# rvp-group/srrg2_proslam

Measured on AMD Instinct MI355X. Metric: tracked frames/sec on KITTI-00 stereo (1241x376, ~2k kp); SE(3) vs ref, higher is better.
Workload: dtype u64 popcount (Hamming) + f32 (projection, Jacobians, 6x6 normal equations)

## Files before the change

srrg2_proslam_amd/csrc/align.hip:

```cpp
#include "prs_device.h"
#include "prs_host.h"
#include "prs_se3.h"

#include <math.h>
#include <string.h>

#include <type_traits>
#include <vector>

namespace prs {

constexpr int kAlignThreads = 256;
constexpr int kTerms        = 29;
constexpr uint32_t kNoneU32 = 0xffffffffu;
constexpr float kFltMax     = 3.402823466e+38f;

typedef unsigned int au32x4 __attribute__((ext_vector_type(4)));

struct AlignShared {
  float X[16];
  float A[16];
  float Sinv[16];
  float T[16];
  float Tprev[16];
// ... 17 lines not shown

static_assert(offsetof(AlignShared, b) == offsetof(AlignShared, H) + 36 * sizeof(float) && offsetof(AlignShared, chi_in) == offsetof(AlignShared, b) + 6 * sizeof(float) &&
                offsetof(AlignShared, chi_tot) == offsetof(AlignShared, chi_in) + sizeof(float),
              "the summed slots are written through AlignShared::H");

struct FrameCtl {
  int it_align;
  int need_search;
  int done;
  int executed;
  int flags;
  int n_inl, n_out, n_inv;
  int db_ready;
};
constexpr int kModeSplitSearch = 100;
constexpr int kSearchThreads   = 512;

struct AlignArgs {
  prs_pcf_params f;
  prs_aligner_params a;
  prs_align_batch b;
  int mode;
  int no_prefilter;
  int surv_slots;
  int narrow_prefilter_limit;
  int rows_table;
  int lut_cap;
  int cell_sy, cell_sx, cell_ncx, cell_ncy, ncells;
  float4* ops;
  FrameCtl* ctl;
  int* pending;
  unsigned char* dbcache;
  uint32_t db_blob;
  unsigned long long* stamps;
  int max_fixed;
  uint32_t off_db, off_inv, off_cellstart, off_cfix, off_cmov, off_cls, off_sh;
  const float* prior_mean;
  uint32_t off_u;
  uint32_t off_fdesc, off_fuv, off_best, off_second, off_lut, off_surv;
  uint32_t off_terms;
};

enum { kDecisionCommit = 0, kDecisionRetry = 1, kDecisionReturn = 2 };



__device__ __forceinline__ int isqrt_exact(int n) {
  int s = (int) sqrtf((float) n);
  while (s * s > n) {
    --s;
  }
  while ((s + 1) * (s + 1) <= n) {
    ++s;
  }
  return s;
}

__device__ __forceinline__ int hamming_regs(const au32x4& a0, const au32x4& a1, const au32x4& b0, const au32x4& b1) {
  uint32_t d = (uint32_t) __popc(a0.x ^ b0.x);
  d = popc_acc(a0.y ^ b0.y, d);
  d = popc_acc(a0.z ^ b0.z, d);
  d = popc_acc(a0.w ^ b0.w, d);
  d = popc_acc(a1.x ^ b1.x, d);
  d = popc_acc(a1.y ^ b1.y, d);
  d = popc_acc(a1.z ^ b1.z, d);
  d = popc_acc(a1.w ^ b1.w, d);
  return (int) d;
}

__device__ __forceinline__ int cold_copy(int v) {
  asm volatile("" : "+v"(v));
  return v;
}

__device__ __forceinline__ int hamming_half(const au32x4& a0, const au32x4& b0) {
  uint32_t d = (uint32_t) __popc(a0.x ^ b0.x);
  d = popc_acc(a0.y ^ b0.y, d);
  d = popc_acc(a0.z ^ b0.z, d);
  d = popc_acc(a0.w ^ b0.w, d);
  return (int) d;
}
__device__ __forceinline__ int hamming_96(const au32x4& a0, const au32x4& b0) {
  uint32_t d = (uint32_t) __popc(a0.x ^ b0.x);
  d = popc_acc(a0.y ^ b0.y, d);
  d = popc_acc(a0.z ^ b0.z, d);
  return (int) d;
}

__device__ __forceinline__ int irrelevant_distance(const float dd, const float ratio) {
  if (!(dd > 0.0f) || !(ratio > 0.0f) || !(dd <= 256.0f)) {
    return 0;
  }
  const int r_max = (int) ceilf(dd) - 1;
  if (r_max <= 0) {
    return 1;
  }
  float guess = (float) r_max / ratio;
  int b       = guess < 1024.0f ? (int) guess : 1024;
  b           = b > r_max ? b : r_max + 1;
  while (b < 2048 && !((float) r_max / (float) b < ratio)) {
    ++b;
  }
  return b < 2048 ? b : 0;
}

// ... 330 lines not shown
    sh.chi_in = sh.chi_tot = 0.0f;
    sh.mean_disp           = (split_search && ctl->it_align != 0) ? gres->mean_disparity : g.a.mean_disparity;
    sh.corr_changed        = 1;
    sh.have_terms          = 0;
    sh.have_cls            = 0;
    if (sh.n_corr < 0 || sh.n_corr > nF) {
      sh.n_corr = 0;
    }
    {
      float x[16], a16[16], si[16];
      const float* gx = g.b.X + (size_t) frame * 16;
#pragma unroll
      for (int i = 0; i < 16; ++i) {
        x[i] = gx[i];
      }
      se3_inverse(g.a.sensor_in_robot, si);
      pose_to_camera(g.a, si, x, a16);
#pragma unroll
      for (int i = 0; i < 16; ++i) {
        sh.Sinv[i] = si[i];
        sh.A[i]    = a16[i];
      }
    }
    if (nF > g.max_fixed) {
      sh.error = PRS_ERR_CAPACITY;
    }
  }
  for (int i = tid; i < 36; i += T) {
    sh.H[i] = 0.0f;
  }
  if (tid < 6) {
    sh.b[tid] = 0.0f;
  }
  __syncthreads();

  bool inputs_changed = g.b.inputs_changed ? (g.b.inputs_changed[frame] != 0) : true;
  if (split_search && ctl->it_align != 0) {
    inputs_changed = false;
  }
  bool db_built       = false;
  if (inputs_changed && g.mode != PRS_MODE_LINEARIZE) {
    if (tid == 0) {
      sh.n_corr = 0;
    }
    __syncthreads();
  }

  if (g.mode != PRS_MODE_FINDER && (!split_search || ctl->it_align == 0) && g.a.factor_type == PRS_FACTOR_STEREO &&
      g.a.enable_inverse_depth_weighting && g.a.mean_disparity < 0.0f && !sh.error) {
    for (int i = tid; i < nF; i += T) {
      const float4 c = gfix[i];
      terms[i]       = c.x - c.z;
    }
    __syncthreads();
    if (tid == 0) {
      float acc = 0.0f;
      int i     = 0;
      const float4* t4 = reinterpret_cast<const float4*>(terms);
      float4 n0 = t4[0], n1 = t4[1], n2 = t4[2], n3 = t4[3];
      for (; i + 16 <= nF; i += 16) {
        const float4 q0 = n0, q1 = n1, q2 = n2, q3 = n3;
        const int k = (i >> 2) + 4;
        n0 = t4[k];
        n1 = t4[k + 1];
        n2 = t4[k + 2];
        n3 = t4[k + 3];
        acc += q0.x; acc += q0.y; acc += q0.z; acc += q0.w;
        acc += q1.x; acc += q1.y; acc += q1.z; acc += q1.w;
        acc += q2.x; acc += q2.y; acc += q2.z; acc += q2.w;
        acc += q3.x; acc += q3.y; acc += q3.z; acc += q3.w;
      }
      for (; i < nF; ++i) {
        acc += terms[i];
      }
      sh.mean_disp = nF > 0 ? acc / (float) (size_t) nF : 0.0f;
    }
    __syncthreads();
  }

  if (g.mode != PRS_MODE_FINDER && !split_search && !sh.error) {
    for (int c = tid; c < sh.n_corr; c += T) {
      const prs_corr cr = gcorr[c];
      if (cr.fixed_idx < 0 || cr.fixed_idx >= nF || cr.moving_idx < 0 || cr.moving_idx >= nM) {
        sh.error = PRS_ERR_RANGE;
      } else {
        cfix[c] = gfix[cr.fixed_idx];
        cmov[c] = gmov[cr.moving_idx];
      }
    }
    __syncthreads();
  }

  enum { acc_finder = 0, acc_lin, acc_sum, acc_solve, acc_db, acc_search, acc_pass2, acc_filter, acc_commit };
  if (g.stamps && tid == 0) {
    for (int i = 0; i < 9; ++i) {
      sh.stamp_acc[i] = 0;
    }
    sh.stamp_mark = sh.stamp_sub = 0;
  }
#define SUB_MARK() do { if (g.stamps && tid == 0) { sh.stamp_sub = (unsigned long long) clock64(); } } while (0)
#define SUB_ACC(v) do { if (g.stamps && tid == 0) { const unsigned long long now_ = (unsigned long long) clock64(); sh.stamp_acc[v] += now_ - sh.stamp_sub; sh.stamp_sub = now_; } } while (0)
#define ALIGN_MARK() do { if (g.stamps && tid == 0) { sh.stamp_mark = (unsigned long long) clock64(); } } while (0)
#define ALIGN_ACC(v) do { if (g.stamps && tid == 0) { sh.stamp_acc[v] += (unsigned long long) clock64() - sh.stamp_mark; } } while (0)
  const int max_it = (g.mode == PRS_MODE_ALIGN && !sh.error) ? g.a.max_iterations + inlier_run_length(g.a) : (sh.error ? 0 : 1);
  if (split_search && sh.error && tid == 0) {
    ctl->done = 1;
  }
  int executed     = 0;
  int it_align     = 0;
  bool ran_inlier_phase = false;
// ... 9 lines not shown
    ALIGN_MARK();
    if (g.mode != PRS_MODE_LINEARIZE && !inlier_run) {
      if (tid < 16) {
        sh.T[tid] = sh.A[tid];
      }
      __syncthreads();
      for (;;) {
        const bool reset = inputs_changed || sh.config_changed;
        __syncthreads();
        if (reset) {
          if (tid == 0) {
            if ((sh.radius == 0 && sh.dd == 0.0f) || sh.config_changed) {
              sh.radius = g.f.maximum_search_radius_pixels;
              sh.dd     = g.f.minimum_descriptor_distance;
            }
            if (sh.config_changed) {
              sh.no_prune = 0;
            }
            sh.converged = 0;
            sh.it        = 0;
            se3_identity(sh.Tprev);
            sh.config_changed = 0;
            sh.kd_range       = (float) sh.radius;
          }
          inputs_changed = false;
          db_built       = false;
          __syncthreads();
        }
        if (sh.error) {
          break;
        }

        if (tid == 0) {
          sh.decision = kDecisionCommit;
          if (sh.converged) {
            sh.decision = kDecisionReturn;
          } else {
            float cam[16];
            se3_inverse(sh.T, cam);
            const unsigned long long k = g.f.number_of_solver_iterations_per_projection;
            if (k == 0 || sh.it % k == 0 || sh.it == 1) {
              se3_inverse(cam, sh.W);
              float delta[16], v6[6];
              se3_mul(cam, sh.Tprev, delta);
              t2tnq(delta, v6);
              sh.change_norm =
                sqrtf(((((v6[0] * v6[0] + v6[1] * v6[1]) + v6[2] * v6[2]) + v6[3] * v6[3]) + v6[4] * v6[4]) + v6[5] * v6[5]);
#pragma unroll
              for (int i = 0; i < 16; ++i) {
                sh.Tprev[i] = sh.T[i];
              }
              sh.n_projected = 0;
              sh.n_overflow  = 0;
              ++sh.num_recomputes;
            } else {
#pragma unroll
              for (int i = 0; i < 16; ++i) {
                sh.Tprev[i] = sh.T[i];
              }
              ++sh.it;
              sh.decision = kDecisionReturn;
            }
          }
        }
        __syncthreads();
        if (sh.decision == kDecisionReturn) {
          break;
        }

        SUB_MARK();
        if (!db_built && split_search && g.dbcache && ctl->db_ready) {
          const uint4* src = reinterpret_cast<const uint4*>(g.dbcache + (size_t) frame * g.db_blob);
          uint4* dst       = reinterpret_cast<uint4*>(smem + g.off_db);
          for (int i = tid; i < (int) (g.db_blob >> 4); i += T) {
            dst[i] = src[i];
          }
          __syncthreads();
          db_built = true;
        }
        if (!db_built && !lattice) {
          const int tid = cold_copy(tid_hot), lane = tid & 63, wave = tid >> 6;
          (void) lane;
          (void) wave;
          KdNode* nodes        = reinterpret_cast<KdNode*>(db);
          uint16_t* order      = inv;
          short* kdhead        = reinterpret_cast<short*>(cellstart);
          uint16_t* leaf_start = cellstart + 2;
          const int node_cap   = (int) ((size_t) g.max_fixed * sizeof(uint2) / sizeof(KdNode));
          const int open_cap   = kd_open_capacity(g.max_fixed);
          const int min_points = g.f.minimum_number_of_points_per_cluster > 0 ? g.f.minimum_number_of_points_per_cluster : 10;
          unsigned long long* st = reinterpret_cast<unsigned long long*>(terms);
          int* cnt        = reinterpret_cast<int*>(st + (size_t) open_cap * 5);
          int* kind       = cnt + open_cap;
          int* child_open = kind + open_cap;
          int* par_cur    = child_open + open_cap;
          int* pcnt_cur   = par_cur + open_cap;
          int* par_next   = pcnt_cur + open_cap;
          int* pcnt_next  = par_next + open_cap;
          uint16_t* node_of = reinterpret_cast<uint16_t*>(pcnt_next + open_cap);
          uint16_t* leaf_of = node_of + g.max_fixed + 2;
          uint16_t* bucket  = leaf_of + g.max_fixed + 2;
          for (int i = tid; i < nF; i += T) {
            const float4 c = gfix[i];
// ... 158 lines not shown
          __syncthreads();
          for (int i = tid; i < nF; i += T) {
            bucket[leaf_start[leaf_of[i]] + node_of[i]] = (uint16_t) i;
          }
          __syncthreads();
          for (int i = tid; i < nF; i += T) {
            const int l0 = leaf_start[leaf_of[i]], l1 = leaf_start[leaf_of[i] + 1];
            int rank = 0;
            for (int j = l0; j < l1; ++j) {
              rank += bucket[j] < (uint16_t) i ? 1 : 0;
            }
            order[l0 + rank] = (uint16_t) i;
          }
          if (tid == 0) {
            kdhead[1] = (short) n_leaves;
          }
          __syncthreads();
          db_built = true;
          if (split_search && g.dbcache) {
            const uint4* src = reinterpret_cast<const uint4*>(smem + g.off_db);
            uint4* dst       = reinterpret_cast<uint4*>(g.dbcache + (size_t) frame * g.db_blob);
            for (int i = tid; i < (int) (g.db_blob >> 4); i += T) {
              dst[i] = src[i];
            }
            if (tid == 0) {
              ctl->db_ready = 1;
            }
          }
        }
        if (!db_built) {
          const int tid = cold_copy(tid_hot), lane = tid & 63, wave = tid >> 6;
          (void) lane;
          (void) wave;
          const int histcap  = (R > g.ncells ? R : g.ncells) + 2;
          uint32_t* hist     = reinterpret_cast<uint32_t*>(terms);
          uint16_t* slot     = reinterpret_cast<uint16_t*>(hist + histcap);
          uint16_t* bucket   = slot + g.max_fixed + 2;
          uint16_t* canon    = bucket + g.max_fixed + 2;
          uint16_t* rowfirst = canon + g.max_fixed + 2;
          for (int i = tid; i <= R; i += T) {
            hist[i] = 0;
          }
          __syncthreads();
          for (int i = tid; i < nF; i += T) {
            const float4 c = gfix[i];
            if (c.x >= 0.0f && c.x < 32767.0f && c.y >= 0.0f && c.y < (float) R) {
              const int row = (int) (int16_t) c.y;
              slot[i]       = (uint16_t) atomicAdd(&hist[row], 1u);
            } else {
              sh.error = PRS_ERR_RANGE;
            }
          }
          __syncthreads();
          if (sh.error) {
            break;
          }
          {
            if (wave == 0) {
              const int n     = R + 1;
              const int chunk = (n + 63) >> 6;
              uint32_t sum    = 0;
              for (int j = 0; j < chunk; ++j) {
                const int r = lane * chunk + j;
                sum += r < n ? hist[r] : 0u;
              }
              uint32_t incl = sum;
#pragma unroll
              for (int d = 1; d < 64; d <<= 1) {
                const uint32_t o = __shfl_up(incl, d, 64);
                if (lane >= d) {
                  incl += o;
                }
              }
              uint32_t run = incl - sum;
              for (int j = 0; j < chunk; ++j) {
                const int r = lane * chunk + j;
                if (r < n) {
                  rowfirst[r] = (uint16_t) run;
                  run += hist[r];
                }
              }
            }
            __syncthreads();
            for (int i = tid; i < nF; i += T) {
              const int row = (int) (int16_t) gfix[i].y;
              bucket[rowfirst[row] + slot[i]] = (uint16_t) i;
            }
            __syncthreads();
            for (int i = tid; i < nF; i += T) {
              const int row = (int) (int16_t) gfix[i].y;
              const int s = rowfirst[row], e = rowfirst[row + 1];
              int rank = 0;
              for (int j = s; j < e; ++j) {
                rank += bucket[j] < (uint16_t) i ? 1 : 0;
              }
              canon[i] = (uint16_t) (s + rank);
            }
          }
          __syncthreads();
          for (int i = tid; i <= g.ncells; i += T) {
            hist[i] = 0;
          }
          __syncthreads();
          for (int i = tid; i < nF; i += T) {
            const float4 c = gfix[i];
            const int row  = (int) (int16_t) c.y;
            int cxi        = ((int) (int16_t) c.x) >> g.cell_sx;
            cxi            = cxi < g.cell_ncx ? cxi : g.cell_ncx - 1;
            slot[i]        = (uint16_t) atomicAdd(&hist[(row >> g.cell_sy) * g.cell_ncx + cxi], 1u);
          }
          __syncthreads();
          if (wave == 0) {
            const int n     = g.ncells + 1;
            const int chunk = (n + 63) >> 6;
            uint32_t sum    = 0;
            for (int j = 0; j < chunk; ++j) {
              const int r = lane * chunk + j;
              sum += r < n ? hist[r] : 0u;
            }
            uint32_t incl = sum;
#pragma unroll
            for (int d = 1; d < 64; d <<= 1) {
              const uint32_t o = __shfl_up(incl, d, 64);
              if (lane >= d) {
                incl += o;
              }
            }
            uint32_t run = incl - sum;
            for (int j = 0; j < chunk; ++j) {
              const int r = lane * chunk + j;
              if (r < n) {
                cellstart[r] = (uint16_t) run;
                run += hist[r];
              }
            }
          }
          __syncthreads();
          for (int i = tid; i < nF; i += T) {
            const float4 c = gfix[i];
            const int row  = (int) (int16_t) c.y;
            const int col  = (int) (int16_t) c.x;
            int cxi        = col >> g.cell_sx;
            cxi            = cxi < g.cell_ncx ? cxi : g.cell_ncx - 1;
            db[cellstart[(row >> g.cell_sy) * g.cell_ncx + cxi] + slot[i]] =
              make_uint2(((uint32_t) row & 0xffffu) | ((uint32_t) col << 16), (uint32_t) i | ((uint32_t) canon[i] << 16));
            inv[canon[i]] = (uint16_t) i;
          }
          if (tid == 0) {
            db[nF] = make_uint2(0x7fff7fffu, 0xffffffffu);
          }
          __syncthreads();
          db_built = true;
          if (split_search && g.dbcache) {
            const uint4* src = reinterpret_cast<const uint4*>(smem + g.off_db);
            uint4* dst       = reinterpret_cast<uint4*>(g.dbcache + (size_t) frame * g.db_blob);
            for (int i = tid; i < (int) (g.db_blob >> 4); i += T) {
              dst[i] = src[i];
            }
            if (tid == 0) {
              ctl->db_ready = 1;
            }
          }
        }

        SUB_ACC(acc_db);
        const int rad = (int) sh.radius;
        {
          const int tid = cold_copy(tid_hot);
          for (int i = tid; i < nF; i += T) {
            bestkey[i] = kNoneU32;
            second[i]  = kNoneU32;
          }
          if (lattice) {
            for (int pos = tid; pos < nF; pos += T) {
              const int fi  = (int) (db[pos].y & 0xffffu);
              fdesc[pos]    = gfd[2 * fi];
              fdesc_hi[pos] = gfd[2 * fi + 1];
            }
          } else {
            for (int i = tid; i < 2 * nF; i += T) {
              (i & 1 ? fdesc_hi : fdesc)[i >> 1] = gfd[i];
            }
            for (int i = tid; i < nF; i += T) {
              const float4 c = gfix[i];
              fuv[i]         = make_float2(c.x, c.y);
            }
          }
          if (stype == PRS_SEARCH_CIRCLE) {
            for (int i = tid; i < 2 * rad + 1 && i < g.lut_cap; i += T) {
              const int h = i - rad;
              lut[i]      = (uint16_t) (isqrt_exact(rad * rad - h * h) + 1);
            }
          }
        }
        __syncthreads();
        SUB_ACC(acc_pass2);
        {
          const float W0 = sh.W[0], W1 = sh.W[1], W2 = sh.W[2], W3 = sh.W[3];
          const float W4 = sh.W[4], W5 = sh.W[5], W6 = sh.W[6], W7 = sh.W[7];
          const float W8 = sh.W[8], W9 = sh.W[9], W10 = sh.W[10], W11 = sh.W[11];
          const float cols = (float) g.f.projector.canvas_cols, rows = (float) g.f.projector.canvas_rows;
          const float max_dd = g.f.maximum_descriptor_distance;
          const float r2f    = (float) (sh.radius * sh.radius);
          const int rad2     = rad * rad;
          const int irrelevant = irrelevant_distance(sh.dd, g.f.maximum_distance_ratio_to_second_best);
          const int prune_at   = (lattice && irrelevant > 0 && irrelevant <= 54 && !g.no_prefilter && !sh.no_prune) ? irrelevant : 0;
          const bool circle_exact = rad < 8192 && R + rad < 32000 && (g.cell_ncx << g.cell_sx) + rad < 32000;
          int projected      = 0;
          constexpr int kPre = SPLIT ? 1 : 4;
          for (int m0 = tid; m0 < nM; m0 += kPre * T) {
// ... 188 lines not shown
              if (bestk != kNoneU32) {
                cd.x = (lattice ? (uint32_t) inv[bestk & 0xffffu] : (bestk & 0xffffu)) | ((bestk >> 16) << 16);
                if (lattice && seck != kNoneU32) {
                  cd.y = (uint32_t) inv[seck & 0xffffu] | ((seck >> 16) << 16);
                }
              }
              auto emit = [&](const uint32_t c, const uint32_t tag) {
                const uint32_t f   = c & 0xffffu;
                const uint32_t key = ((c >> 16) << 17) | ((uint32_t) m << 1) | tag;
                const uint32_t old = atomicMin(&bestkey[f], key);
                if (old != kNoneU32) {
                  atomicMin(&second[f], (old > key ? old : key) >> 17);
                }
              };
              if (cd.x != kNoneU32) {
                emit(cd.x, 0u);
              }
              if (cd.y != kNoneU32) {
                emit(cd.y, 1u);
              }
            }
           }
          }
          if (projected) {
            atomicAdd(&sh.n_projected, projected);
          }
        }
        __syncthreads();
        SUB_ACC(acc_search);
        {
          const float ratio = g.f.maximum_distance_ratio_to_second_best;
          const float dd    = sh.dd;
          int base          = 0;
          for (int f0 = 0; f0 < nF; f0 += T) {
            const int f = f0 + tid;
            bool acc    = false;
            if (f < nF) {
              const uint32_t bk = bestkey[f];
              if (bk != kNoneU32) {
                const float resp = (float) (bk >> 17);
                const uint32_t s = second[f];
                const float fs   = s == kNoneU32 ? kFltMax : (float) s;
                acc = resp < dd && resp / fs < ratio && (bk & 1u) == 0u;
              }
            }
            const unsigned long long bal = __ballot(acc);
            const int pre                = __popcll(bal & ((1ull << lane) - 1ull));
            if (lane == 0) {
              sh.wave_tot[wave] = __popcll(bal);
            }
            __syncthreads();
            int wbase = base;
            for (int w = 0; w < wave; ++w) {
              wbase += sh.wave_tot[w];
            }
            if (f < nF) {
              second[f] = acc ? (uint32_t) (wbase + pre) : kNoneU32;
            }
            for (int w = 0; w < T / 64; ++w) {
              base += sh.wave_tot[w];
            }
            __syncthreads();
          }
          if (tid == 0) {
            sh.n_filtered = base;
          }
        }
        __syncthreads();
        if (tid == 0) {
          if (sh.n_projected == 0) {
            sh.flags |= PRS_WARN_NO_PROJECTION;
          }
          if (8 * sh.n_overflow > sh.n_projected) {
            sh.no_prune = 1;
          }
          const float matching_ratio = (float) sh.n_filtered / (float) (size_t) nF;
          sh.decision                = kDecisionCommit;
          if (matching_ratio < g.f.minimum_matching_ratio) {
            sh.flags |= PRS_WARN_LOW_RATIO;
            if (sh.radius < g.f.maximum_search_radius_pixels || sh.dd > g.f.minimum_descriptor_distance) {
              sh.radius = g.f.maximum_search_radius_pixels;
              sh.dd     = g.f.minimum_descriptor_distance;
              sh.flags |= PRS_WARN_RETRIED;
              if (matching_ratio == 0.0f) {
                sh.flags |= PRS_WARN_TRACK_LOST;
                se3_identity(sh.T);
                sh.it = 0;
              } else {
                ++sh.it;
              }
              sh.decision = kDecisionRetry;
            }
          }
          if (sh.decision == kDecisionCommit) {
            sh.n_corr       = sh.n_filtered;
            sh.corr_changed = 1;
            if (sh.change_norm < g.f.maximum_estimate_change_norm_for_convergence &&
                sh.it > g.f.minimum_number_of_iterations) {
              sh.converged = 1;
              if (matching_ratio > g.f.minimum_matching_ratio) {
                const unsigned long long reduced = sh.radius - g.f.search_radius_step_size_pixels;
                sh.radius = reduced > g.f.minimum_search_radius_pixels ? reduced : g.f.minimum_search_radius_pixels;
                const float increased = sh.dd + g.f.descriptor_distance_step_size_pixels;
                sh.dd = increased < g.f.maximum_descriptor_distance ? increased : g.f.maximum_descriptor_distance;
              }
            }
            ++sh.it;
          }
        }
        __syncthreads();
        if (sh.decision == kDecisionRetry) {
          continue;
        }
        SUB_ACC(acc_filter);
        for (int f = cold_copy(tid_hot); f < nF; f += T) {
          const uint32_t slot = second[f];
          if (slot != kNoneU32) {
            const uint32_t bk = bestkey[f];
            const int m       = (int) ((bk >> 1) & 0xffffu);
            prs_corr cr;
            cr.fixed_idx  = f;
            cr.moving_idx = m;
            cr.response   = (float) (bk >> 17);
            gcorr[slot]   = cr;
            if (g.mode == PRS_MODE_ALIGN) {
              cfix[slot] = gfix[f];
              cmov[slot] = gmov[m];
            }
          }
        }
        __syncthreads();
        SUB_ACC(acc_commit);
        break;
      }
      if (sh.error) {
        break;
      }
      if (tid == 0 && sh.n_corr == 0) {
        sh.flags |= PRS_WARN_NO_MATCHES;
      }
      __syncthreads();
    }
    ALIGN_ACC(acc_finder);
    if (g.mode == PRS_MODE_FINDER || split_search) {
      break;
    }

    const int nc = sh.n_corr;
    __syncthreads();
    if (g.mode == PRS_MODE_ALIGN && nc < g.a.min_num_correspondences) {
      if (tid == 0) {
        sh.n_inl = sh.n_out = sh.n_inv = 0;
        sh.chi_in = sh.chi_tot = 0.0f;
        sh.have_cls = 0;
      }
      for (int i = tid; i < 36; i += T) {
        sh.H[i] = 0.0f;
      }
      if (tid < 6) {
        sh.b[tid] = 0.0f;
      }
      __syncthreads();
      if (g.a.stop_at_fixed_point && (sh.converged || inlier_run)) {
        ran_inlier_phase = ran_inlier_phase || (inlier_run_length(g.a) > 0 && 0 >= g.a.min_num_inliers);
        break;
      }
      continue;
    }
    {
      const PoseRegs pose  = {sh.A[0], sh.A[1], sh.A[2], sh.A[3], sh.A[4], sh.A[5], sh.A[6], sh.A[7], sh.A[8], sh.A[9], sh.A[10], sh.A[11]};
      const float mean_dsp = sh.mean_disp;
      const bool pose_ok   = __all(pose_is_finite(pose));
      if (tid == 0) {
        sh.have_cls = 1;
// ... 86 lines not shown
      if (g.a.enable_motion_prior) {
        add_motion_prior(g.a, g.prior_mean ? g.prior_mean + (size_t) frame * 16 : nullptr, X, H, b);
      }
      float dx6[6];
      const bool step_ok = gn_step(H, b, g.a.damping, X, g.a.damping_form == PRS_DAMPING_IDENTITY, dx6);
      const float dn2 = ((((dx6[0] * dx6[0] + dx6[1] * dx6[1]) + dx6[2] * dx6[2]) + dx6[3] * dx6[3]) + dx6[4] * dx6[4]) + dx6[5] * dx6[5];
      const bool small_step = g.a.step_norm_exit > 0.0f && step_ok && dn2 < g.a.step_norm_exit * g.a.step_norm_exit;
      uint32_t changed_bits = 0;
#pragma unroll
      for (int i = 0; i < 16; ++i) {
        changed_bits |= __float_as_uint(X[i]) ^ __float_as_uint(sh.X[i]);
        sh.X[i] = X[i];
      }
      float a16[16];
      pose_to_camera(g.a, sh.Sinv, X, a16);
#pragma unroll
      for (int i = 0; i < 16; ++i) {
        sh.A[i] = a16[i];
      }
      sh.decision = ((g.a.stop_at_fixed_point && changed_bits == 0u && (sh.converged || inlier_run)) || (small_step && (sh.converged || inlier_run))) ? 1 : 0;
    }
    __syncthreads();
    ALIGN_ACC(acc_solve);
    if (sh.decision) {
      if (!inlier_run && inlier_run_length(g.a) > 0) {
        it_align = g.a.max_iterations - 1;
        continue;
      }
      ++it_align;
      break;
    }
  }

  __syncthreads();
  if (g.mode == PRS_MODE_ALIGN && !split_search && g.a.keep_only_inlier_correspondences && sh.have_cls && !sh.error) {
    const int nc = sh.n_corr;
    int base     = 0;
    for (int c0 = 0; c0 < nc; c0 += T) {
      const int c     = c0 + tid;
      const bool keep = c < nc && clsbuf[c] == 0;
      prs_corr cr;
      if (keep) {
        cr = gcorr[c];
      }
      const unsigned long long bal = __ballot(keep);
      if (lane == 0) {
        sh.wave_tot[wave] = __popcll(bal);
      }
      __syncthreads();
      int pos = base + __popcll(bal & ((1ull << lane) - 1ull));
      for (int w = 0; w < T / 64; ++w) {
        pos += w < wave ? sh.wave_tot[w] : 0;
        base += sh.wave_tot[w];
      }
      if (keep) {
        gcorr[pos] = cr;
      }
      __syncthreads();
    }
    if (tid == 0) {
      sh.n_corr = base;
    }
    __syncthreads();
  }

  __syncthreads();
  if (tid < 16) {
    if (!split_search) {
      g.b.X[(size_t) frame * 16 + tid] = sh.X[tid];
    }
    gstate->local_map_in_sensor[tid]          = sh.T[tid];
    gstate->local_map_in_sensor_previous[tid] = sh.Tprev[tid];
  }
  for (int i = tid; i < 36; i += T) {
    gres->H[i] = sh.H[i];
  }
  if (tid < 6) {
    gres->b[tid] = sh.b[tid];
  }
  if (tid == 0) {
    gstate->search_radius_pixels = sh.radius;
    gstate->current_iteration    = sh.it;
    gstate->descriptor_distance  = sh.dd;
    gstate->database_leaf_range  = sh.kd_range;
    gstate->has_converged        = sh.converged;
    gstate->config_changed       = sh.config_changed;
    gstate->num_recomputes       = sh.num_recomputes;
    gstate->reserved             = (gstate->reserved & ~1) | sh.no_prune;
    g.b.n_corr[frame]            = sh.n_corr;
    gres->chi_inliers            = sh.chi_in;
    gres->chi_total              = sh.chi_tot;
    gres->mean_disparity         = sh.mean_disp;
    gres->num_inliers            = sh.n_inl;
    gres->num_outliers           = sh.n_out;
    gres->num_invalid            = sh.n_inv;
    gres->num_correspondences    = sh.n_corr;
    gres->status                 = sh.n_inl >= g.a.min_num_inliers ? 1 : 0;
    gres->iterations             = g.mode == PRS_MODE_ALIGN ? (ran_inlier_phase ? max_it : g.a.max_iterations) : 1;
    gres->iterations_executed    = executed;
// ... 522 lines not shown
    r.num_inliers = r.num_outliers = r.num_invalid = r.num_correspondences = 0;
    r.status = r.iterations = r.iterations_executed = r.warnings = 0;
    res[i]                                                        = r;
  }
  if (i == 0) {
    *pending = 0;
  }
}

__global__ void gn_step_kernel(const float* H, const float* b, float damping, int identity_damping, float* X, int* ok) {
  float h[36], bb[6], x[16];
  for (int i = 0; i < 36; ++i) {
    h[i] = H[i];
  }
  for (int i = 0; i < 6; ++i) {
    bb[i] = b[i];
  }
  for (int i = 0; i < 16; ++i) {
    x[i] = X[i];
  }
  const bool r = gn_step(h, bb, damping, x, identity_damping != 0);
  for (int i = 0; i < 16; ++i) {
    X[i] = x[i];
  }
  *ok = r ? 1 : 0;
}

static inline uint32_t align_up16(uint32_t v) {
  return (v + 15u) / 16u * 16u;
}

struct SplitJob {
  bool active = false;
  void* own[3]        = {nullptr, nullptr, nullptr};
  size_t own_bytes[3] = {0, 0, 0};
  hipStream_t stream  = nullptr;
  hipStream_t capture_stream = nullptr;
  ~SplitJob() {
    for (void* p : own) {
      if (p) {
        (void) hipFree(p);
      }
    }
  }
  void* buffer(hipStream_t s, int i, size_t bytes) {
    if (bytes <= own_bytes[i]) {
      return own[i];
    }
    if (own[i]) {
      (void) hipStreamSynchronize(s);
      (void) hipFree(own[i]);
      own[i]       = nullptr;
      own_bytes[i] = 0;
    }
    const size_t want = bytes + bytes / 4 + 4096;
    if (hipMalloc(&own[i], want) != hipSuccess) {
      own[i] = nullptr;
      return nullptr;
    }
    own_bytes[i] = want;
    return own[i];
  }
  AlignArgs g, gs;
  void (*search)(AlignArgs) = nullptr;
  void (*gn)(AlignArgs)     = nullptr;
  size_t lds_search = 0, lds_gn = 0;
  int total = 0, limit = 0;
  int enqueued = 0;
// ... 63 lines not shown
  while (cells_of(sy, sx, ncy, ncx) > 2048) {
    if (ncy > ncx) {
      ++sy;
    } else {
      ++sx;
    }
  }
  g.cell_sy  = sy;
  g.cell_sx  = sx;
  g.cell_ncy = ncy;
  g.cell_ncx = ncx;
  g.ncells   = ncy * ncx;
  const bool kdtree         = finder->search_type == PRS_SEARCH_KDTREE;
  const uint32_t cs_entries = kdtree && nf + 4u > (uint32_t) g.ncells + 2u ? nf + 4u : (uint32_t) g.ncells + 2u;
  auto carve = [&](AlignArgs& g, bool with_operands) -> size_t {
    uint32_t off = 0;
    g.off_db       = off; off = align_up16(off + (nf + 1) * 8);
    g.off_inv      = off; off = align_up16(off + nf * 2);
    g.off_cellstart = off; off = align_up16(off + cs_entries * 2);
    g.off_cfix     = off; off = align_up16(off + (with_operands ? nf * 16 : 0));
    g.off_cmov     = off; off = align_up16(off + (with_operands ? nf * 16 : 0));
    g.off_cls      = off; off = align_up16(off + (with_operands ? nf : 0));
    g.off_sh       = off; off = align_up16(off + (uint32_t) sizeof(AlignShared));
    g.off_u        = off;
    uint32_t u = off;
    g.off_fdesc  = u; u = align_up16(u + nf * 32);
    g.off_fuv    = u; u = align_up16(u + (finder->search_type == PRS_SEARCH_KDTREE ? nf * 8 : 0));
    g.off_best   = u; u = align_up16(u + nf * 4);
    g.off_second = u; u = align_up16(u + nf * 4);
    g.off_lut    = u; u = align_up16(u + lut_cap * 2);
    g.off_surv   = u; u = align_up16(u + (uint32_t) (with_operands ? kAlignThreads : kSearchThreads) * (uint32_t) g.surv_slots * 2);
    g.off_terms = off;
    uint32_t terms_bytes       = kTerms * kAlignThreads * 4;
    const uint32_t histcap     = (R > (uint32_t) g.ncells ? R : (uint32_t) g.ncells) + 2;
    const uint32_t build_bytes = histcap * 4 + (nf + 2) * 2 * 3 + (R + 2) * 2 + 16;
    if (build_bytes > terms_bytes) {
      terms_bytes = build_bytes;
    }
    if (nf * 4 + 160 > terms_bytes) {
      terms_bytes = nf * 4 + 160;
    }
    const uint32_t kd_bytes = (uint32_t) kd_open_capacity((int) nf) * (40 + 7 * 4) + (nf + 2) * 2 * 3 + 64;
    if (kdtree && kd_bytes > terms_bytes) {
      terms_bytes = kd_bytes;
    }
    const uint32_t t_end = align_up16(off + terms_bytes);
    return u > t_end ? u : t_end;
  };
  g.surv_slots     = 4;
  const size_t lds = carve(g, true);
  if (lds > 160 * 1024) {
    return ctx_fail(ctx, PRS_ERR_UNSUPPORTED, "prs_align_batch_run: fixed cloud does not fit the 160 KiB LDS (lower max_fixed)");
  }
  g.stamps = ctx_stamps(ctx, (size_t) batch->batch * 16 * sizeof(unsigned long long));
  g.ops     = nullptr;
  g.ctl     = nullptr;
  g.pending = nullptr;
  g.dbcache = nullptr;
  g.db_blob = 0;
  hipStream_t stream = ctx_stream(ctx);
  hipError_t e;
  if (max_fixed >= (int) kClsOutUnit) {
    return ctx_fail(ctx, PRS_ERR_UNSUPPORTED, "prs_align_batch_run: max_fixed must be below 2048");
  }
  const bool stamps_split = g.stamps && ctx->stamps_split;
  const bool split = mode == PRS_MODE_ALIGN && !ctx_fused_align(ctx) && max_fixed <= kGnThreads * kGnSlots && (!g.stamps || stamps_split);
  if (!split) {
    auto kernel = align_kernel<kAlignThreads, false, -1>;
    e           = hipFuncSetAttribute(reinterpret_cast<const void*>(kernel), hipFuncAttributeMaxDynamicSharedMemorySize, (int) lds);
    if (e != hipSuccess) {
      return ctx_fail_hip(ctx, e, "prs_align_batch_run attribute");
    }
    hipLaunchKernelGGL(kernel, dim3(batch->batch), dim3(kAlignThreads), lds, stream, g);
    e = hipGetLastError();
    if (e != hipSuccess) {
      return ctx_fail_hip(ctx, e, "prs_align_batch_run launch");
    }
    if (g.stamps) {
      ctx_report_stamps(ctx, batch->batch, 10, "align (fused, 256 threads): finder | linearize + in-wave reduction | cross-wave sum | GN solve || of finder: lattice build | projection+search | staging (keys, fixed rows -> LDS) | filter | commit");
    }
    return PRS_OK;
  }
  SplitJob* job = static_cast<SplitJob*>(ctx->align_job);
  if (!job) {
    job                 = new SplitJob();
    ctx->align_job      = job;
    ctx->align_job_free = [](void* p) { delete static_cast<SplitJob*>(p); };
  }
  const size_t ops_bytes = (size_t) batch->batch * (size_t) max_fixed * 2 * sizeof(float4);
  const size_t ctl_bytes = (size_t) batch->batch * sizeof(FrameCtl) + 256;
  unsigned char* small   = static_cast<unsigned char*>(job->buffer(stream, 0, ctl_bytes));
  g.ops                  = static_cast<float4*>(job->buffer(stream, 1, ops_bytes));
  if (!small || !g.ops) {
    return ctx_fail(ctx, PRS_ERR_HIP, "prs_align_batch_run: split-pipeline scratch allocation failed");
  }
  g.pending = reinterpret_cast<int*>(small);
  g.ctl     = reinterpret_cast<FrameCtl*>(small + 256);
  AlignArgs gs = g;
  gs.mode      = kModeSplitSearch;
  gs.surv_slots = 8;
  size_t lds_search = carve(gs, false);
  gs.surv_slots     = 4;
  {
    const size_t lds4 = carve(gs, false);
    if ((160u * 1024u) / lds_search == (160u * 1024u) / lds4 && finder->search_type != PRS_SEARCH_KDTREE) {
      gs.surv_slots = 8;
      lds_search    = carve(gs, false);
    } else {
      lds_search = lds4;
    }
  }
  gs.db_blob = align_up16(gs.off_cellstart + cs_entries * 2) - gs.off_db;
  gs.dbcache = static_cast<unsigned char*>(job->buffer(stream, 2, (size_t) batch->batch * gs.db_blob));
  if (!gs.dbcache) {
    return ctx_fail(ctx, PRS_ERR_HIP, "prs_align_batch_run: lattice cache allocation failed");
  }
  const bool wide_slots = gs.surv_slots == 8;
  auto skernel = finder->search_type == PRS_SEARCH_CIRCLE
                   ? (wide_slots ? align_kernel<kSearchThreads, true, PRS_SEARCH_CIRCLE, 8> : align_kernel<kSearchThreads, true, PRS_SEARCH_CIRCLE, 4>)
                   : (finder->search_type == PRS_SEARCH_SQUARE
                        ? (wide_slots ? align_kernel<kSearchThreads, true, PRS_SEARCH_SQUARE, 8> : align_kernel<kSearchThreads, true, PRS_SEARCH_SQUARE, 4>)
                        : (finder->search_type == PRS_SEARCH_RHOMBUS
                             ? (wide_slots ? align_kernel<kSearchThreads, true, PRS_SEARCH_RHOMBUS, 8> : align_kernel<kSearchThreads, true, PRS_SEARCH_RHOMBUS, 4>)
                             : align_kernel<kSearchThreads, true, PRS_SEARCH_KDTREE, 4>));
  e = hipFuncSetAttribute(reinterpret_cast<const void*>(skernel), hipFuncAttributeMaxDynamicSharedMemorySize, (int) lds_search);
  if (e != hipSuccess) {
    return ctx_fail_hip(ctx, e, "prs_align_batch_run attribute");
  }
  hipLaunchKernelGGL(split_init_kernel, dim3((batch->batch + 255) / 256), dim3(256), 0, stream, g.ctl, batch->result, g.pending, batch->batch);
  const bool fast = aligner->factor_type == PRS_FACTOR_STEREO && !aligner->keep_only_inlier_correspondences && aligner->kernel_weight_form == PRS_KERNEL_WEIGHT_INV_CHI &&
                    aligner->damping_form == PRS_DAMPING_DIAG && aligner->translation_weight_form == PRS_TRANSLATION_WEIGHT_OFFSET;
  int n_cu = 0;
  (void) hipDeviceGetAttribute(&n_cu, hipDeviceAttributeMultiprocessorCount, ctx->device);
  const bool lone = fast && batch->batch <= 2 * (n_cu > 0 ? n_cu : 256) && !ctx->no_lone_gn;
  const bool five = fast && !lone && max_fixed > 4 * 128;
  const bool lean  = !batch->prior && !aligner->with_sensor && !aligner->enable_inlier_only_runs;
  const bool plain = lean && !aligner->enable_motion_prior;
  const bool mprior = lean && aligner->enable_motion_prior;
  const bool depth = aligner->factor_type == PRS_FACTOR_DEPTH && aligner->kernel_weight_form == PRS_KERNEL_WEIGHT_INV_CHI && aligner->damping_form == PRS_DAMPING_DIAG;
  auto gnk        = lone ? (max_fixed <= 4 * 128 ? (plain ? gn_kernel<4, PRS_FACTOR_STEREO, false, kGnLdsSlots, 1, 1> : gn_kernel<4, PRS_FACTOR_STEREO, false, kGnLdsSlots, 1>)
                                                 : (plain ? gn_kernel<8, PRS_FACTOR_STEREO, false, kGnLdsSlots, 1, 1> : gn_kernel<8, PRS_FACTOR_STEREO, false, kGnLdsSlots, 1>))
                         : (max_fixed <= 4 * 128 ? (fast ? (plain ? gn_kernel<4, PRS_FACTOR_STEREO, false, kGnLdsSlots, 4, 1> : (mprior ? gn_kernel<4, PRS_FACTOR_STEREO, false, kGnLdsSlots, 4, 2> : gn_kernel<4, PRS_FACTOR_STEREO, false>))
                                                         : (depth ? gn_kernel<4, PRS_FACTOR_DEPTH, true> : gn_kernel<4, 0, true>))
                                                 : (fast ? (plain ? gn_kernel<8, PRS_FACTOR_STEREO, false, 3, 5, 1> : (mprior ? gn_kernel<8, PRS_FACTOR_STEREO, false, 3, 5, 2> : gn_kernel<8, PRS_FACTOR_STEREO, false, 3, 5>))
                                                         : (depth ? gn_kernel<8, PRS_FACTOR_DEPTH, true> : gn_kernel<8, 0, true>)));
  const size_t lds_gn = gn_lds_bytes(five ? 3 : kGnLdsSlots);
  job->active      = true;
  job->stream      = stream;
// ... 160 lines not shown
```

Before: 1.762 million.

## Cache lattice-ordered descriptors, fuse lattice build histograms, and trim barriers in split search

Adds a per-frame global cache of descriptors in lattice order, so later split-search iterations reload the LDS database and descriptor rows in one pass instead of regathering them. The lattice build now fills the row and cell histograms in one pass, scans both with a block-wide DPP scan, and folds the mean-disparity reduction into the same pass using exact fixed-point sums. The filter compaction handles two chunks per barrier, and several trailing __syncthreads are skipped in split mode. These cut serial work and barriers, at the cost of an extra global buffer, more LDS scratch and more complex ordering logic.

```diff
diff --git a/srrg2_proslam_amd/csrc/align.hip b/srrg2_proslam_amd/csrc/align.hip
--- a/srrg2_proslam_amd/csrc/align.hip
+++ b/srrg2_proslam_amd/csrc/align.hip
@@ -73,6 +73,7 @@
   int* pending;
   unsigned char* dbcache;
   uint32_t db_blob;
+  au32x4* rowcache;
   unsigned long long* stamps;
   int max_fixed;
   uint32_t off_db, off_inv, off_cellstart, off_cfix, off_cmov, off_cls, off_sh;
@@ -112,6 +113,39 @@
 __device__ __forceinline__ int cold_copy(int v) {
   asm volatile("" : "+v"(v));
   return v;
+}
+
+__device__ __forceinline__ uint32_t wave_inclusive_scan_dpp(uint32_t v) {
+  v += (uint32_t) __builtin_amdgcn_update_dpp(0, (int) v, 0x111, 0xf, 0xf, true);
+  v += (uint32_t) __builtin_amdgcn_update_dpp(0, (int) v, 0x112, 0xf, 0xf, true);
+  v += (uint32_t) __builtin_amdgcn_update_dpp(0, (int) v, 0x114, 0xf, 0xf, true);
+  v += (uint32_t) __builtin_amdgcn_update_dpp(0, (int) v, 0x118, 0xf, 0xf, true);
+  v += (uint32_t) __builtin_amdgcn_update_dpp(0, (int) v, 0x142, 0xa, 0xf, false);
+  v += (uint32_t) __builtin_amdgcn_update_dpp(0, (int) v, 0x143, 0xc, 0xf, false);
+  return v;
+}
+
+__device__ __forceinline__ float serial_float_sum(const float* col, const int n) {
+  float acc = 0.0f;
+  int i     = 0;
+  const float4* t4 = reinterpret_cast<const float4*>(col);
+  float4 n0 = t4[0], n1 = t4[1], n2 = t4[2], n3 = t4[3];
+  for (; i + 16 <= n; i += 16) {
+    const float4 q0 = n0, q1 = n1, q2 = n2, q3 = n3;
+    const int k = (i >> 2) + 4;
+    n0 = t4[k];
+    n1 = t4[k + 1];
+    n2 = t4[k + 2];
+    n3 = t4[k + 3];
+    acc += q0.x; acc += q0.y; acc += q0.z; acc += q0.w;
+    acc += q1.x; acc += q1.y; acc += q1.z; acc += q1.w;
+    acc += q2.x; acc += q2.y; acc += q2.z; acc += q2.w;
+    acc += q3.x; acc += q3.y; acc += q3.z; acc += q3.w;
+  }
+  for (; i < n; ++i) {
+    acc += col[i];
+  }
+  return acc;
 }
 
 __device__ __forceinline__ int hamming_half(const au32x4& a0, const au32x4& b0) {
@@ -508,13 +542,38 @@
   if (tid < 6) {
     sh.b[tid] = 0.0f;
   }
+  bool db_built = false;
+  if (split_search && lattice && g.rowcache && ctl->db_ready && ctl->it_align != 0 && nF <= g.max_fixed) {
+    const uint4* __restrict__ img   = reinterpret_cast<const uint4*>(g.dbcache + (size_t) frame * g.db_blob);
+    const au32x4* __restrict__ rows = g.rowcache + (size_t) frame * 2 * (size_t) g.max_fixed;
+    uint4* dst      = reinterpret_cast<uint4*>(smem + g.off_db);
+    const int n_img = (int) (g.db_blob >> 4);
+    for (int i = tid; i < (n_img > nF ? n_img : nF); i += T) {
+      uint4 a   = make_uint4(0u, 0u, 0u, 0u);
+      au32x4 lo = {0u, 0u, 0u, 0u}, hi = {0u, 0u, 0u, 0u};
+      if (i < n_img) {
+        a = img[i];
+      }
+      if (i < nF) {
+        lo = rows[i];
+        hi = rows[g.max_fixed + i];
+      }
+      if (i < n_img) {
+        dst[i] = a;
+      }
+      if (i < nF) {
+        fdesc[i]    = lo;
+        fdesc_hi[i] = hi;
+      }
+    }
+    db_built = true;
+  }
   __syncthreads();
 
   bool inputs_changed = g.b.inputs_changed ? (g.b.inputs_changed[frame] != 0) : true;
   if (split_search && ctl->it_align != 0) {
     inputs_changed = false;
   }
-  bool db_built       = false;
   if (inputs_changed && g.mode != PRS_MODE_LINEARIZE) {
     if (tid == 0) {
       sh.n_corr = 0;
@@ -522,36 +581,23 @@
     __syncthreads();
   }
 
-  if (g.mode != PRS_MODE_FINDER && (!split_search || ctl->it_align == 0) && g.a.factor_type == PRS_FACTOR_STEREO &&
-      g.a.enable_inverse_depth_weighting && g.a.mean_disparity < 0.0f && !sh.error) {
+  const auto binds_disparity = [&]() {
+    return g.mode != PRS_MODE_FINDER && (!split_search || ctl->it_align == 0) && g.a.factor_type == PRS_FACTOR_STEREO && g.a.enable_inverse_depth_weighting &&
+           g.a.mean_disparity < 0.0f;
+  };
+  const auto bind_disparity = [&]() {
     for (int i = tid; i < nF; i += T) {
       const float4 c = gfix[i];
       terms[i]       = c.x - c.z;
     }
     __syncthreads();
     if (tid == 0) {
-      float acc = 0.0f;
-      int i     = 0;
-      const float4* t4 = reinterpret_cast<const float4*>(terms);
-      float4 n0 = t4[0], n1 = t4[1], n2 = t4[2], n3 = t4[3];
-      for (; i + 16 <= nF; i += 16) {
-        const float4 q0 = n0, q1 = n1, q2 = n2, q3 = n3;
-        const int k = (i >> 2) + 4;
-        n0 = t4[k];
-        n1 = t4[k + 1];
-        n2 = t4[k + 2];
-        n3 = t4[k + 3];
-        acc += q0.x; acc += q0.y; acc += q0.z; acc += q0.w;
-        acc += q1.x; acc += q1.y; acc += q1.z; acc += q1.w;
-        acc += q2.x; acc += q2.y; acc += q2.z; acc += q2.w;
-        acc += q3.x; acc += q3.y; acc += q3.z; acc += q3.w;
-      }
-      for (; i < nF; ++i) {
-        acc += terms[i];
-      }
-      sh.mean_disp = nF > 0 ? acc / (float) (size_t) nF : 0.0f;
+      sh.mean_disp = nF > 0 ? serial_float_sum(terms, nF) / (float) (size_t) nF : 0.0f;
     }
     __syncthreads();
+  };
+  if (!(split_search && lattice) && binds_disparity() && !sh.error) {
+    bind_disparity();
   }
 
   if (g.mode != PRS_MODE_FINDER && !split_search && !sh.error) {
@@ -627,6 +673,9 @@
         }
 
         if (tid == 0) {
+          if (nF == 0 || nM == 0) {
+            sh.flags |= PRS_WARN_EMPTY_INPUT;
+          }
           sh.decision = kDecisionCommit;
           if (sh.converged) {
             sh.decision = kDecisionReturn;
@@ -664,6 +713,7 @@
         }
 
         SUB_MARK();
+        const bool stage_rows = !split_search || !db_built;
         if (!db_built && split_search && g.dbcache && ctl->db_ready) {
           const uint4* src = reinterpret_cast<const uint4*>(g.dbcache + (size_t) frame * g.db_blob);
           uint4* dst       = reinterpret_cast<uint4*>(smem + g.off_db);
@@ -888,23 +938,63 @@
           const int tid = cold_copy(tid_hot), lane = tid & 63, wave = tid >> 6;
           (void) lane;
           (void) wave;
-          const int histcap  = (R > g.ncells ? R : g.ncells) + 2;
-          uint32_t* hist     = reinterpret_cast<uint32_t*>(terms);
-          uint16_t* slot     = reinterpret_cast<uint16_t*>(hist + histcap);
-          uint16_t* bucket   = slot + g.max_fixed + 2;
-          uint16_t* canon    = bucket + g.max_fixed + 2;
-          uint16_t* rowfirst = canon + g.max_fixed + 2;
+          constexpr int kWaves = T / 64;
+          static_assert(2 * kWaves <= 16, "AlignShared::wave_tot holds the wave totals of both scans");
+          float* disp         = terms;
+          uint32_t* hist_row  = reinterpret_cast<uint32_t*>(disp + g.max_fixed + 40);
+          uint32_t* hist_cell = hist_row + R + 2;
+          uint32_t* rowcol    = hist_cell + g.ncells + 2;
+          int* dsum           = reinterpret_cast<int*>(rowcol + g.max_fixed);
+          uint16_t* slot      = reinterpret_cast<uint16_t*>(dsum + 4);
+          uint16_t* cslot     = slot + g.max_fixed + 2;
+          uint16_t* bucket    = cslot + g.max_fixed + 2;
+          uint16_t* rowfirst  = bucket + g.max_fixed + 2;
+          const bool bind     = split_search && binds_disparity();
           for (int i = tid; i <= R; i += T) {
-            hist[i] = 0;
+            hist_row[i] = 0;
+          }
+          for (int i = tid; i <= g.ncells; i += T) {
+            hist_cell[i] = 0;
+          }
+          if (tid == 0) {
+            dsum[0] = dsum[1] = dsum[2] = 0;
           }
           __syncthreads();
+          int msum = 0, mabs = 0;
+          bool inexact = false;
           for (int i = tid; i < nF; i += T) {
             const float4 c = gfix[i];
+            if (bind) {
+              const float d = c.x - c.z;
+              const float q = d * 16.0f;
+              const bool ok = __builtin_fabsf(q) < 1048576.0f && q == __builtin_rintf(q);
+              const int m   = ok ? (int) q : 0;
+              disp[i]       = d;
+              msum += m;
+              mabs += m < 0 ? -m : m;
+              inexact = inexact || !ok;
+            }
             if (c.x >= 0.0f && c.x < 32767.0f && c.y >= 0.0f && c.y < (float) R) {
               const int row = (int) (int16_t) c.y;
-              slot[i]       = (uint16_t) atomicAdd(&hist[row], 1u);
+              const int col = (int) (int16_t) c.x;
+              int cxi       = col >> g.cell_sx;
+              cxi           = cxi < g.cell_ncx ? cxi : g.cell_ncx - 1;
+              rowcol[i]     = ((uint32_t) row & 0xffffu) | ((uint32_t) col << 16);
+              slot[i]       = (uint16_t) atomicAdd(&hist_row[row], 1u);
+              cslot[i]      = (uint16_t) atomicAdd(&hist_cell[(row >> g.cell_sy) * g.cell_ncx + cxi], 1u);
             } else {
               sh.error = PRS_ERR_RANGE;
+            }
+          }
+          if (bind) {
+            const uint32_t wsum = wave_inclusive_scan_dpp((uint32_t) msum), wabs = wave_inclusive_scan_dpp((uint32_t) mabs);
+            const bool winexact = __ballot(inexact) != 0ull;
+            if (lane == 63) {
+              atomicAdd(&dsum[0], (int) wsum);
+              atomicAdd(&dsum[1], (int) wabs);
+              if (winexact) {
+                dsum[2] = 1;
+              }
             }
           }
           __syncthreads();
@@ -912,95 +1002,66 @@
             break;
           }
           {
-            if (wave == 0) {
-              const int n     = R + 1;
-              const int chunk = (n + 63) >> 6;
-              uint32_t sum    = 0;
-              for (int j = 0; j < chunk; ++j) {
-                const int r = lane * chunk + j;
-                sum += r < n ? hist[r] : 0u;
+            const int chunk_r = (R + T) / T, chunk_c = (g.ncells + T) / T;
+            uint32_t sum_r = 0, sum_c = 0;
+            for (int j = 0; j < chunk_r; ++j) {
+              const int r = tid * chunk_r + j;
+              sum_r += r <= R ? hist_row[r] : 0u;
+            }
+            for (int j = 0; j < chunk_c; ++j) {
+              const int r = tid * chunk_c + j;
+              sum_c += r <= g.ncells ? hist_cell[r] : 0u;
+            }
+            const uint32_t incl_r = wave_inclusive_scan_dpp(sum_r), incl_c = wave_inclusive_scan_dpp(sum_c);
+            if (lane == 63) {
+              sh.wave_tot[wave]          = (int) incl_r;
+              sh.wave_tot[kWaves + wave] = (int) incl_c;
+            }
+            if (bind && tid == T - 64) {
+              const bool exact = !dsum[2] && dsum[1] < (1 << 24);
+              const float acc  = exact ? (float) dsum[0] * 0.0625f : serial_float_sum(disp, nF);
+              sh.mean_disp     = nF > 0 ? acc / (float) (size_t) nF : 0.0f;
+            }
+            __syncthreads();
+            uint32_t run_r = incl_r - sum_r, run_c = incl_c - sum_c;
+#pragma unroll
+            for (int w = 0; w < kWaves; ++w) {
+              run_r += w < wave ? (uint32_t) sh.wave_tot[w] : 0u;
+              run_c += w < wave ? (uint32_t) sh.wave_tot[kWaves + w] : 0u;
+            }
+            for (int j = 0; j < chunk_r; ++j) {
+              const int r = tid * chunk_r + j;
+              if (r <= R) {
+                rowfirst[r] = (uint16_t) run_r;
+                run_r += hist_row[r];
               }
-              uint32_t incl = sum;
-#pragma unroll
-              for (int d = 1; d < 64; d <<= 1) {
-                const uint32_t o = __shfl_up(incl, d, 64);
-                if (lane >= d) {
-                  incl += o;
-                }
+            }
+            for (int j = 0; j < chunk_c; ++j) {
+              const int r = tid * chunk_c + j;
+              if (r <= g.ncells) {
+                cellstart[r] = (uint16_t) run_c;
+                run_c += hist_cell[r];
               }
-              uint32_t run = incl - sum;
-              for (int j = 0; j < chunk; ++j) {
-                const int r = lane * chunk + j;
-                if (r < n) {
-                  rowfirst[r] = (uint16_t) run;
-                  run += hist[r];
-                }
-              }
-            }
-            __syncthreads();
-            for (int i = tid; i < nF; i += T) {
-              const int row = (int) (int16_t) gfix[i].y;
-              bucket[rowfirst[row] + slot[i]] = (uint16_t) i;
-            }
-            __syncthreads();
-            for (int i = tid; i < nF; i += T) {
-              const int row = (int) (int16_t) gfix[i].y;
-              const int s = rowfirst[row], e = rowfirst[row + 1];
-              int rank = 0;
-              for (int j = s; j < e; ++j) {
-                rank += bucket[j] < (uint16_t) i ? 1 : 0;
-              }
-              canon[i] = (uint16_t) (s + rank);
-            }
-          }
-          __syncthreads();
-          for (int i = tid; i <= g.ncells; i += T) {
-            hist[i] = 0;
+            }
           }
           __syncthreads();
           for (int i = tid; i < nF; i += T) {
-            const float4 c = gfix[i];
-            const int row  = (int) (int16_t) c.y;
-            int cxi        = ((int) (int16_t) c.x) >> g.cell_sx;
-            cxi            = cxi < g.cell_ncx ? cxi : g.cell_ncx - 1;
-            slot[i]        = (uint16_t) atomicAdd(&hist[(row >> g.cell_sy) * g.cell_ncx + cxi], 1u);
-          }
-          __syncthreads();
-          if (wave == 0) {
-            const int n     = g.ncells + 1;
-            const int chunk = (n + 63) >> 6;
-            uint32_t sum    = 0;
-            for (int j = 0; j < chunk; ++j) {
-              const int r = lane * chunk + j;
-              sum += r < n ? hist[r] : 0u;
-            }
-            uint32_t incl = sum;
-#pragma unroll
-            for (int d = 1; d < 64; d <<= 1) {
-              const uint32_t o = __shfl_up(incl, d, 64);
-              if (lane >= d) {
-                incl += o;
-              }
-            }
-            uint32_t run = incl - sum;
-            for (int j = 0; j < chunk; ++j) {
-              const int r = lane * chunk + j;
-              if (r < n) {
-                cellstart[r] = (uint16_t) run;
-                run += hist[r];
-              }
-            }
+            bucket[rowfirst[rowcol[i] & 0xffffu] + slot[i]] = (uint16_t) i;
           }
           __syncthreads();
           for (int i = tid; i < nF; i += T) {
-            const float4 c = gfix[i];
-            const int row  = (int) (int16_t) c.y;
-            const int col  = (int) (int16_t) c.x;
-            int cxi        = col >> g.cell_sx;
-            cxi            = cxi < g.cell_ncx ? cxi : g.cell_ncx - 1;
-            db[cellstart[(row >> g.cell_sy) * g.cell_ncx + cxi] + slot[i]] =
-              make_uint2(((uint32_t) row & 0xffffu) | ((uint32_t) col << 16), (uint32_t) i | ((uint32_t) canon[i] << 16));
-            inv[canon[i]] = (uint16_t) i;
+            const uint32_t rc = rowcol[i];
+            const int row = (int) (rc & 0xffffu), col = (int) (rc >> 16);
+            const int s = rowfirst[row], e = rowfirst[row + 1];
+            int rank = 0;
+            for (int j = s; j < e; ++j) {
+              rank += bucket[j] < (uint16_t) i ? 1 : 0;
+            }
+            const int canon = s + rank;
+            int cxi         = col >> g.cell_sx;
+            cxi             = cxi < g.cell_ncx ? cxi : g.cell_ncx - 1;
+            db[cellstart[(row >> g.cell_sy) * g.cell_ncx + cxi] + cslot[i]] = make_uint2(rc, (uint32_t) i | ((uint32_t) canon << 16));
+            inv[canon]                                                      = (uint16_t) i;
           }
           if (tid == 0) {
             db[nF] = make_uint2(0x7fff7fffu, 0xffffffffu);
@@ -1028,10 +1089,18 @@
             second[i]  = kNoneU32;
           }
           if (lattice) {
-            for (int pos = tid; pos < nF; pos += T) {
-              const int fi  = (int) (db[pos].y & 0xffffu);
-              fdesc[pos]    = gfd[2 * fi];
-              fdesc_hi[pos] = gfd[2 * fi + 1];
+            if (stage_rows) {
+              au32x4* rows = split_search && g.rowcache ? g.rowcache + (size_t) frame * 2 * (size_t) g.max_fixed : nullptr;
+              for (int pos = tid; pos < nF; pos += T) {
+                const int fi    = (int) (db[pos].y & 0xffffu);
+                const au32x4 lo = gfd[2 * fi], hi = gfd[2 * fi + 1];
+                fdesc[pos]      = lo;
+                fdesc_hi[pos]   = hi;
+                if (rows) {
+                  rows[pos]               = lo;
+                  rows[g.max_fixed + pos] = hi;
+                }
+              }
             }
           } else {
             for (int i = tid; i < 2 * nF; i += T) {
@@ -1286,41 +1355,59 @@
           const float ratio = g.f.maximum_distance_ratio_to_second_best;
           const float dd    = sh.dd;
           int base          = 0;
-          for (int f0 = 0; f0 < nF; f0 += T) {
-            const int f = f0 + tid;
-            bool acc    = false;
-            if (f < nF) {
-              const uint32_t bk = bestkey[f];
-              if (bk != kNoneU32) {
-                const float resp = (float) (bk >> 17);
-                const uint32_t s = second[f];
-                const float fs   = s == kNoneU32 ? kFltMax : (float) s;
-                acc = resp < dd && resp / fs < ratio && (bk & 1u) == 0u;
+          constexpr int kWaves = T / 64;
+          static_assert(2 * kWaves <= 16, "AlignShared::wave_tot holds the wave totals of two chunks");
+          for (int f0 = 0; f0 < nF; f0 += 2 * T) {
+            if (f0 != 0) {
+              __syncthreads();
+            }
+            bool acc[2];
+            int pre[2];
+#pragma unroll
+            for (int k = 0; k < 2; ++k) {
+              const int f = f0 + k * T + tid;
+              acc[k]      = false;
+              if (f < nF) {
+                const uint32_t bk = bestkey[f];
+                if (bk != kNoneU32) {
+                  const float resp = (float) (bk >> 17);
+                  const uint32_t s = second[f];
+                  const float fs   = s == kNoneU32 ? kFltMax : (float) s;
+                  acc[k] = resp < dd && resp / fs < ratio && (bk & 1u) == 0u;
+                }
               }
-            }
-            const unsigned long long bal = __ballot(acc);
-            const int pre                = __popcll(bal & ((1ull << lane) - 1ull));
-            if (lane == 0) {
-              sh.wave_tot[wave] = __popcll(bal);
+              const unsigned long long bal = __ballot(acc[k]);
+              pre[k]                       = __popcll(bal & ((1ull << lane) - 1ull));
+              if (lane == 0) {
+                sh.wave_tot[k * kWaves + wave] = __popcll(bal);
+              }
             }
             __syncthreads();
-            int wbase = base;
-            for (int w = 0; w < wave; ++w) {
-              wbase += sh.wave_tot[w];
-            }
-            if (f < nF) {
-              second[f] = acc ? (uint32_t) (wbase + pre) : kNoneU32;
-            }
-            for (int w = 0; w < T / 64; ++w) {
-              base += sh.wave_tot[w];
-            }
-            __syncthreads();
+            int wbase[2] = {0, 0};
+            int run      = base;
+#pragma unroll
+            for (int j = 0; j < 2 * kWaves; ++j) {
+              if (j == wave) {
+                wbase[0] = run;
+              }
+              if (j == kWaves + wave) {
+                wbase[1] = run;
+              }
+              run += sh.wave_tot[j];
+            }
+            base = run;
+#pragma unroll
+            for (int k = 0; k < 2; ++k) {
+              const int f = f0 + k * T + tid;
+              if (f < nF) {
+                second[f] = acc[k] ? (uint32_t) (wbase[k] + pre[k]) : kNoneU32;
+              }
+            }
           }
           if (tid == 0) {
             sh.n_filtered = base;
           }
         }
-        __syncthreads();
         if (tid == 0) {
           if (sh.n_projected == 0) {
             sh.flags |= PRS_WARN_NO_PROJECTION;
@@ -1383,7 +1470,9 @@
             }
           }
         }
-        __syncthreads();
+        if (!split_search || g.stamps) {
+          __syncthreads();
+        }
         SUB_ACC(acc_commit);
         break;
       }
@@ -1393,7 +1482,9 @@
       if (tid == 0 && sh.n_corr == 0) {
         sh.flags |= PRS_WARN_NO_MATCHES;
       }
-      __syncthreads();
+      if (!split_search) {
+        __syncthreads();
+      }
     }
     ALIGN_ACC(acc_finder);
     if (g.mode == PRS_MODE_FINDER || split_search) {
@@ -1546,7 +1637,9 @@
     }
   }
 
-  __syncthreads();
+  if (!split_search) {
+    __syncthreads();
+  }
   if (g.mode == PRS_MODE_ALIGN && !split_search && g.a.keep_only_inlier_correspondences && sh.have_cls && !sh.error) {
     const int nc = sh.n_corr;
     int base     = 0;
@@ -1578,7 +1671,13 @@
     __syncthreads();
   }
 
-  __syncthreads();
+  if (split_search && lattice && !db_built && binds_disparity() && sh.error != PRS_ERR_CAPACITY) {
+    bind_disparity();
+  }
+
+  if (!split_search) {
+    __syncthreads();
+  }
   if (tid < 16) {
     if (!split_search) {
       g.b.X[(size_t) frame * 16 + tid] = sh.X[tid];
@@ -2167,8 +2266,8 @@
 
 struct SplitJob {
   bool active = false;
-  void* own[3]        = {nullptr, nullptr, nullptr};
-  size_t own_bytes[3] = {0, 0, 0};
+  void* own[4]        = {nullptr, nullptr, nullptr, nullptr};
+  size_t own_bytes[4] = {0, 0, 0, 0};
   hipStream_t stream  = nullptr;
   hipStream_t capture_stream = nullptr;
   ~SplitJob() {
@@ -2298,13 +2397,9 @@
     g.off_surv   = u; u = align_up16(u + (uint32_t) (with_operands ? kAlignThreads : kSearchThreads) * (uint32_t) g.surv_slots * 2);
     g.off_terms = off;
     uint32_t terms_bytes       = kTerms * kAlignThreads * 4;
-    const uint32_t histcap     = (R > (uint32_t) g.ncells ? R : (uint32_t) g.ncells) + 2;
-    const uint32_t build_bytes = histcap * 4 + (nf + 2) * 2 * 3 + (R + 2) * 2 + 16;
+    const uint32_t build_bytes = (nf + 40) * 4 + (R + 2 + (uint32_t) g.ncells + 2) * 4 + nf * 4 + 16 + (nf + 2) * 2 * 3 + (R + 2) * 2 + 16;
     if (build_bytes > terms_bytes) {
       terms_bytes = build_bytes;
-    }
-    if (nf * 4 + 160 > terms_bytes) {
-      terms_bytes = nf * 4 + 160;
     }
     const uint32_t kd_bytes = (uint32_t) kd_open_capacity((int) nf) * (40 + 7 * 4) + (nf + 2) * 2 * 3 + 64;
     if (kdtree && kd_bytes > terms_bytes) {
@@ -2324,6 +2419,7 @@
   g.pending = nullptr;
   g.dbcache = nullptr;
   g.db_blob = 0;
+  g.rowcache = nullptr;
   hipStream_t stream = ctx_stream(ctx);
   hipError_t e;
   if (max_fixed >= (int) kClsOutUnit) {
@@ -2380,6 +2476,13 @@
   gs.dbcache = static_cast<unsigned char*>(job->buffer(stream, 2, (size_t) batch->batch * gs.db_blob));
   if (!gs.dbcache) {
     return ctx_fail(ctx, PRS_ERR_HIP, "prs_align_batch_run: lattice cache allocation failed");
+  }
+  gs.rowcache = nullptr;
+  if (!kdtree) {
+    gs.rowcache = static_cast<au32x4*>(job->buffer(stream, 3, (size_t) batch->batch * (size_t) max_fixed * 2 * sizeof(au32x4)));
+    if (!gs.rowcache) {
+      return ctx_fail(ctx, PRS_ERR_HIP, "prs_align_batch_run: descriptor row cache allocation failed");
+    }
   }
   const bool wide_slots = gs.surv_slots == 8;
   auto skernel = finder->search_type == PRS_SEARCH_CIRCLE
```

Result: faster. 1.786 million, median of 6 (+1.3%).
